# videosegmentation/video_segment

Hardware: AMD Instinct MI355X
Metric: over-segmented frames/sec at 1080p (higher is better)
Workload: dtype f32

## Files before the change

include/vsg.h:

```cpp
#ifndef VSG_H_
#define VSG_H_

#include <stddef.h>
#include <stdint.h>

#ifdef __cplusplus
extern "C" {
#endif

#define VSG_OK 0
#define VSG_ERR_INVALID -1
#define VSG_ERR_DEVICE -2
#define VSG_ERR_STATE -3
#define VSG_ERR_INTERNAL -4

#define VSG_MEM_HOST 0
#define VSG_MEM_DEVICE 1

typedef struct vsg_stream vsg_stream;
typedef struct vsg_graph vsg_graph;

typedef struct vsg_options {
  int presmoothing;
  float frac_min_region_size;
// ... 16 lines not shown
  float readout_ms;
  float host_post_ms;
  int64_t edges_total;
  int64_t edges_active;
  int64_t merges;
  int64_t preprocess_launches;
  int64_t edge_launches;
  float wave_kernel_ms;
  int64_t wave_kernel_launches;
  int64_t wave_kernel_edges;
  float filter_kernel_ms;
  int64_t filter_kernel_launches;
  float spine_kernel_ms;
  int64_t spine_kernel_launches;
  int64_t spine_kernel_edges;
} vsg_timings;

typedef struct vsg_diagnostics {
  double segment_wall_ms;
  double prepare_ms;
  double constrained_merge_ms;
  int64_t stages;
  int64_t optimistic_stages, rollbacks;
  int64_t slab_growths;
  double slab_growth_ms;
  int64_t spine_pool_growths;
  double spine_pool_growth_ms;
  int64_t runtime_mallocs;
  double runtime_malloc_ms;
  int64_t runtime_frees;
  double runtime_free_ms;
  int64_t cache_hits;
  int64_t device_syncs;
  double device_sync_ms;
  int64_t mail_waits;
  double mail_wait_ms;
  double mail_wait_longest_ms;
  int mail_mode;
} vsg_diagnostics;

typedef struct vsg_merge_paths {
  int64_t hub_stages;
  int64_t hub_absorbed;
  int64_t hub_cuts;
  int64_t hub_cuts_in_groups;
  int64_t hub_parts_in_later_bucket;
  int64_t spine_side_cuts;
  int64_t hub_retries;
  int64_t hub_reasons[6];
  int64_t hub_exclusion_reruns;
  int64_t hub_off_reruns;
  int64_t group_halvings;
  int64_t conservative_replays;
} vsg_merge_paths;

typedef struct vsg_memory_stats {
  int64_t bytes_in_use;
  int64_t bytes_in_use_peak;
  int64_t bytes_cached;
  int64_t limit_bytes;
  int64_t runtime_mallocs, runtime_frees, cache_hits, device_syncs;
  double runtime_malloc_ms, runtime_free_ms, device_sync_ms;
} vsg_memory_stats;
int vsg_device_memory_stats(int device, vsg_memory_stats* out);
int vsg_device_memory_trim(int device);
int vsg_device_memory_limit(int device, int64_t bytes);

const char* vsg_last_error(void);
int vsg_version(void);
void vsg_default_options(vsg_options* o);
int vsg_device_count(void);

int vsg_vectorize_id_image(const int32_t* ids, int width, int height, const uint8_t** data,
                           size_t* len);

int vsg_stream_create(const vsg_options* o, int width, int height, vsg_stream** out);
void vsg_stream_destroy(vsg_stream* s);
int vsg_stream_process_frame(vsg_stream* s, int flush, const uint8_t* bgr, size_t stride,
                             const float* flow, int has_flow_stream, int mem, int* num_results);
int vsg_stream_chunk_size(const vsg_stream* s);
int vsg_stream_result_bytes(vsg_stream* s, int i, const uint8_t** data, size_t* len);
int vsg_stream_result_id_image(vsg_stream* s, int i, int32_t* out);
int vsg_stream_last_merge_stats(const vsg_stream* s, int64_t* forced_regular_small);
int vsg_stream_last_timings(const vsg_stream* s, vsg_timings* t);
int vsg_stream_last_diagnostics(const vsg_stream* s, vsg_diagnostics* d);
int vsg_stream_last_merge_paths(const vsg_stream* s, vsg_merge_paths* out);
int vsg_stream_last_smoothed(vsg_stream* s, float* out);

int vsg_stream_export_halo(vsg_stream* s, const int32_t** dev_labels_virtual,
                           const int32_t** dev_labels_constrained, int64_t scalars[4]);
int vsg_stream_import_halo(vsg_stream* s, const int32_t* labels_virtual,
                           const int32_t* labels_constrained, int mem, const int64_t scalars[4]);

int vsg_stream_expect_halo(vsg_stream* s);
int vsg_stream_restart(vsg_stream* s);

typedef struct vsg_chain vsg_chain;
int vsg_chain_create(int rank, int world, const char* id_file, uint64_t nonce, int device,
                     vsg_chain** out);
void vsg_chain_destroy(vsg_chain* c);
int vsg_chain_info(const vsg_chain* c, int* rank, int* world);
int vsg_chain_send_halo(vsg_chain* c, vsg_stream* from, int dst);
int vsg_chain_recv_halo(vsg_chain* c, vsg_stream* into, int src);
int vsg_chain_exchange_halo(vsg_chain* c, vsg_stream* from, int dst, vsg_stream* into, int src);

typedef struct vsg_regionseg vsg_regionseg;
// ... 72 lines not shown
```

video_segment_amd/_lib.py:

```python
import ctypes as C
import os
import subprocess

_HERE = os.path.dirname(os.path.abspath(__file__))
CSRC_DIR = os.path.join(_HERE, "csrc")
LIB_PATH = os.path.join(_HERE, "lib", "libvsg_hip.so")

VSG_OK = 0
VSG_ERR_INVALID, VSG_ERR_DEVICE, VSG_ERR_STATE, VSG_ERR_INTERNAL = -1, -2, -3, -4
VSG_MEM_HOST = 0
VSG_MEM_DEVICE = 1


class VsgOptions(C.Structure):
    _fields_ = [
        ("presmoothing", C.c_int),
        ("frac_min_region_size", C.c_float),
        ("chunk_size", C.c_int),
        ("chunk_overlap_ratio", C.c_float),
        ("num_constraint_frames", C.c_int),
        ("enforce_n4_connectivity", C.c_int),
        ("enforce_spatial_connectedness", C.c_int),
        ("color_distance", C.c_int),
        ("device", C.c_int),
# ... 1 lines not shown
        ("compute_vectorization", C.c_int),
    ]


class VsgTimings(C.Structure):
    _fields_ = [
        ("preprocess_ms", C.c_float),
        ("edges_ms", C.c_float),
        ("sort_ms", C.c_float),
        ("merge_ms", C.c_float),
        ("readout_ms", C.c_float),
        ("host_post_ms", C.c_float),
        ("edges_total", C.c_int64),
        ("edges_active", C.c_int64),
        ("merges", C.c_int64),
        ("preprocess_launches", C.c_int64),
        ("edge_launches", C.c_int64),
        ("wave_kernel_ms", C.c_float),
        ("wave_kernel_launches", C.c_int64),
        ("wave_kernel_edges", C.c_int64),
        ("filter_kernel_ms", C.c_float),
        ("filter_kernel_launches", C.c_int64),
        ("spine_kernel_ms", C.c_float),
        ("spine_kernel_launches", C.c_int64),
        ("spine_kernel_edges", C.c_int64),
    ]


class VsgDiagnostics(C.Structure):
    _fields_ = [
        ("segment_wall_ms", C.c_double), ("prepare_ms", C.c_double), ("constrained_merge_ms", C.c_double),
        ("stages", C.c_int64), ("optimistic_stages", C.c_int64), ("rollbacks", C.c_int64),
        ("slab_growths", C.c_int64), ("slab_growth_ms", C.c_double),
        ("spine_pool_growths", C.c_int64), ("spine_pool_growth_ms", C.c_double),
        ("runtime_mallocs", C.c_int64), ("runtime_malloc_ms", C.c_double),
        ("runtime_frees", C.c_int64), ("runtime_free_ms", C.c_double),
        ("cache_hits", C.c_int64), ("device_syncs", C.c_int64), ("device_sync_ms", C.c_double),
        ("mail_waits", C.c_int64), ("mail_wait_ms", C.c_double), ("mail_wait_longest_ms", C.c_double),
        ("mail_mode", C.c_int),
    ]

    def as_dict(self):
        return {k: getattr(self, k) for k, _ in self._fields_}


class VsgMergePaths(C.Structure):
    _fields_ = [
        ("hub_stages", C.c_int64), ("hub_absorbed", C.c_int64),
        ("hub_cuts", C.c_int64), ("hub_cuts_in_groups", C.c_int64), ("hub_parts_in_later_bucket", C.c_int64),
        ("spine_side_cuts", C.c_int64),
        ("hub_retries", C.c_int64), ("hub_reasons", C.c_int64 * 6),
        ("hub_exclusion_reruns", C.c_int64), ("hub_off_reruns", C.c_int64),
        ("group_halvings", C.c_int64), ("conservative_replays", C.c_int64),
    ]

    def as_dict(self):
        return {k: (list(getattr(self, k)) if k == "hub_reasons" else getattr(self, k)) for k, _ in self._fields_}


class VsgMemoryStats(C.Structure):
    _fields_ = [
        ("bytes_in_use", C.c_int64), ("bytes_in_use_peak", C.c_int64), ("bytes_cached", C.c_int64),
        ("limit_bytes", C.c_int64),
        ("runtime_mallocs", C.c_int64), ("runtime_frees", C.c_int64), ("cache_hits", C.c_int64),
        ("device_syncs", C.c_int64),
        ("runtime_malloc_ms", C.c_double), ("runtime_free_ms", C.c_double), ("device_sync_ms", C.c_double),
    ]

    def as_dict(self):
        return {k: getattr(self, k) for k, _ in self._fields_}


class VsgRegionOptions(C.Structure):
    _fields_ = [
        ("min_region_num", C.c_int), ("max_region_num", C.c_int),
        ("level_cutoff_fraction", C.c_float), ("small_region_penalizer", C.c_float),
        ("luminance_bins", C.c_int), ("color_bins", C.c_int), ("flow_bins", C.c_int),
        ("chunk_set_size", C.c_int), ("chunk_set_overlap", C.c_int), ("constraint_chunks", C.c_int),
        ("use_appearance", C.c_int), ("use_flow", C.c_int), ("use_size_penalizer", C.c_int),
        ("compute_vectorization", C.c_int), ("save_descriptors", C.c_int),
    ]


EXPORTED_SYMBOLS = [
    "vsg_last_error", "vsg_version", "vsg_default_options", "vsg_device_count",
    "vsg_device_memory_stats", "vsg_device_memory_trim", "vsg_device_memory_limit",
    "vsg_vectorize_id_image",
    "vsg_stream_create", "vsg_stream_destroy", "vsg_stream_process_frame", "vsg_stream_chunk_size",
    "vsg_stream_result_bytes", "vsg_stream_result_id_image", "vsg_stream_last_merge_stats",
    "vsg_stream_last_timings", "vsg_stream_last_diagnostics", "vsg_stream_last_merge_paths", "vsg_stream_last_smoothed", "vsg_stream_export_halo",
    "vsg_stream_import_halo", "vsg_stream_expect_halo", "vsg_stream_restart",
    "vsg_chain_create", "vsg_chain_destroy", "vsg_chain_info", "vsg_chain_send_halo",
    "vsg_chain_recv_halo", "vsg_chain_exchange_halo",
    "vsg_regionseg_default_options", "vsg_regionseg_create", "vsg_regionseg_destroy", "vsg_regionseg_process_frame",
    "vsg_regionseg_result_bytes", "vsg_bgr_to_lab",
    "vsg_graph_create", "vsg_graph_destroy", "vsg_graph_add_frame_bgr",
    "vsg_graph_add_frame_features", "vsg_graph_add_virtual_frame", "vsg_graph_add_temporal",
    "vsg_graph_finish_building", "vsg_graph_segment_spatially", "vsg_graph_segment", "vsg_graph_obtain_results",
    "vsg_graph_num_frames", "vsg_graph_num_regions", "vsg_graph_num_neighbor_links",
    "vsg_graph_region_sizes", "vsg_graph_index_image", "vsg_graph_get_regions",
    "vsg_graph_get_intervals", "vsg_graph_smoothed",
    "vsg_graph_spatial_buckets", "vsg_graph_temporal_buckets", "vsg_graph_node_roots",
    "vsg_graph_merge_stats", "vsg_graph_timings", "vsg_graph_diagnostics", "vsg_graph_merge_paths",
    "vsg_debug_sort_pairs", "vsg_debug_sort_pairs_timed",
]

# ... 118 lines not shown
```

video_segment_amd/csrc/capi.cpp:

```cpp
#include <algorithm>
#include <cstring>
#include <memory>
#include <string>
#include <vector>

#include <rccl/rccl.h>

#include <chrono>
#include <cstdio>
#include <fstream>
#include <thread>

#include "../../include/vsg.h"
#include "region_segmentation.h"
#include "stream.h"

namespace {

thread_local std::string g_last_error;

template <class F>
int Guard(F&& f) {
  try {
    f();
// ... 47 lines not shown
}

}

struct vsg_stream {
  int device = 0;
  std::unique_ptr<vsg::DenseSegmentationHip> impl;
  std::vector<int32_t> id_image;
};

struct vsg_regionseg {
  std::unique_ptr<vsg::RegionSegmentationHost> impl;
  int W = 0, H = 0;
};

struct vsg_graph {
  int device = 0;
  int W = 0, H = 0;
  size_t wh = 0;
  hipStream_t stream = nullptr;
  std::unique_ptr<vsg::DenseGraphHip> g;
  std::unique_ptr<vsg::Preprocessor> pre;
  std::vector<std::shared_ptr<vsg::DevBuf<float>>> feats;
  std::vector<std::shared_ptr<vsg::DevBuf<float>>> flows_dev;
  vsg::DevBuf<uint8_t> staging_bgr;
  vsg::DevBuf<float> staging_f32;
  vsg::DevBuf<int32_t> staging_ids;
  vsg_timings timings;
  std::vector<vsg_region> out_regions;
  std::vector<int32_t> out_nbr_ptr, out_nbr_idx;
  std::vector<vsg_interval> out_intervals;
  ~vsg_graph() {
    if (stream) (void)hipStreamSynchronize(stream);
    g.reset();
    pre.reset();
    if (stream) (void)hipStreamDestroy(stream);
  }
};

static void FillMergePaths(const vsg::MergePaths& mp, vsg_merge_paths* o) {
  std::memset(o, 0, sizeof(*o));
  o->hub_stages = mp.hub_stages;
  o->hub_absorbed = mp.hub_absorbed;
  o->hub_cuts = mp.hub_cuts;
  o->hub_cuts_in_groups = mp.hub_cuts_in_groups;
  o->hub_parts_in_later_bucket = mp.hub_parts_in_later_bucket;
  o->spine_side_cuts = mp.spine_side_cuts;
  o->hub_retries = mp.hub_retries;
  for (int q = 0; q < 6; ++q) o->hub_reasons[q] = mp.hub_reasons[q];
  o->hub_exclusion_reruns = mp.hub_exclusion_reruns;
  o->hub_off_reruns = mp.hub_off_reruns;
  o->group_halvings = mp.group_halvings;
  o->conservative_replays = mp.conservative_replays;
}

static void FillDiagnostics(const vsg::GraphTimings& gt, vsg_diagnostics* d) {
  std::memset(d, 0, sizeof(*d));
  d->segment_wall_ms = gt.segment_wall_ms;
  d->prepare_ms = gt.prepare_ms;
  d->constrained_merge_ms = gt.constrained_merge_ms;
  d->stages = gt.stages;
  d->optimistic_stages = gt.optimistic_stages;
  d->rollbacks = gt.rollbacks;
  d->slab_growths = gt.slab_growths;
  d->slab_growth_ms = gt.slab_growth_ms;
  d->spine_pool_growths = gt.spine_growths;
  d->spine_pool_growth_ms = gt.spine_growth_ms;
  d->runtime_mallocs = gt.runtime_mallocs;
  d->runtime_malloc_ms = gt.runtime_malloc_ms;
  d->runtime_frees = gt.runtime_frees;
  d->runtime_free_ms = gt.runtime_free_ms;
  d->cache_hits = gt.cache_hits;
  d->device_syncs = gt.device_syncs;
  d->device_sync_ms = gt.device_sync_ms;
  d->mail_waits = gt.mail_waits;
  d->mail_wait_ms = gt.mail_wait_ms;
  d->mail_wait_longest_ms = gt.mail_wait_longest_ms;
  d->mail_mode = gt.mail_mode;
}

extern "C" {

const char* vsg_last_error(void) { return g_last_error.c_str(); }

int vsg_device_memory_stats(int device, vsg_memory_stats* out) {
  return Guard([&] {
    VSG_REQUIRE(out, VSG_ERR_INVALID, "null argument");
    const int dev = ResolveDevice(device);
    const vsg::CacheStats s = vsg::CacheGetStats(dev);
    out->bytes_in_use = s.bytes_in_use;
    out->bytes_in_use_peak = s.bytes_in_use_peak;
    out->bytes_cached = s.bytes_cached;
    out->limit_bytes = s.limit_bytes;
    out->runtime_mallocs = s.runtime_mallocs;
    out->runtime_frees = s.runtime_frees;
    out->cache_hits = s.cache_hits;
    out->device_syncs = s.device_syncs;
    out->runtime_malloc_ms = s.runtime_malloc_ms;
    out->runtime_free_ms = s.runtime_free_ms;
    out->device_sync_ms = s.device_sync_ms;
  });
}

int vsg_device_memory_trim(int device) {
  return Guard([&] {
    const int dev = ResolveDevice(device);
// ... 858 lines not shown
```

video_segment_amd/csrc/dense_graph.cpp:

```cpp
#include "dense_graph.h"
#include "scan_device.h"

#include <algorithm>
#include <chrono>
#include <cmath>
#include <cstring>
#include <atomic>
#include <functional>
#include <thread>
#include <unordered_set>

namespace vsg {

namespace {
template <class T>
DevBuf<T>& Grow(DevBuf<T>& b, size_t n) {
  if (b.size() < n) b.alloc(n + n / 2 + 1024);
  return b;
}
double NowMs() {
  using clk = std::chrono::steady_clock;
  return std::chrono::duration<double, std::milli>(clk::now().time_since_epoch()).count();
}
template <class T>
// ... 425 lines not shown
    if (getenv("VSG_DEBUG_STATS")) {
      std::fprintf(stderr, "[vsg] stage scratch: %zu -> %zu active edges (needed %lld), %.2f ms\n", before,
                   scratch_active_, need, NowMs() - tg0);
    }
    return true;
  };
  S.num_active = scalars_.get();
  S.num_segs = scalars_.get() + 1;
  S.node_key_bits = 1;
  while (S.node_key_bits < 32 && ((size_t)1 << S.node_key_bits) < N) ++S.node_key_bits;
  {
    const size_t words = 4 * ((scratch_edges_ + 255) / 256) + 4;
    S.masks.active = filter_masks_.get();
    S.masks.settled = filter_masks_.get() + words;
    S.masks.tentative = filter_masks_.get() + 2 * words;
    S.masks.block_cnt = block_cnt_.get();
    S.block_off = block_off_.get();
  }
  S.force_rollback = getenv("VSG_FORCE_ROLLBACK") ? 1 : 0;
  S.small_seg = getenv("VSG_SMALL_SEG") ? std::max(1, atoi(getenv("VSG_SMALL_SEG"))) : 24;
  S.wide_min = getenv("VSG_WIDE_MIN") ? atoi(getenv("VSG_WIDE_MIN")) : 0;
  S.wide_waves = getenv("VSG_WIDE_WAVES") ? atoi(getenv("VSG_WIDE_WAVES")) : 4;
  S.chain_relax = getenv("VSG_CHAIN_RELAX") ? atoi(getenv("VSG_CHAIN_RELAX")) : 1;
  const int hubs_default = getenv("VSG_HUBS") ? atoi(getenv("VSG_HUBS")) : 1;
  S.hubs = hubs_default;
  S.hub_excl = hub_excl_.get();
  S.hub_max_splits = getenv("VSG_HUB_SPLITS") ? std::max(0, atoi(getenv("VSG_HUB_SPLITS"))) : kHubMaxSplits;
  S.hub_cut_min_work = getenv("VSG_CUT_MIN_WORK") ? atoi(getenv("VSG_CUT_MIN_WORK")) : 0;
  S.hub_cut_ratio = getenv("VSG_CUT_RATIO") ? std::max(0, atoi(getenv("VSG_CUT_RATIO"))) : 1500;
  S.hub_check = (getenv("VSG_HUB_CHECK") && atoi(getenv("VSG_HUB_CHECK")) != 0) ? 1 : 0;
  VSG_HIP(hipMemsetAsync(hub8_.get(), 0, N, stream_));
  S.spine_min = getenv("VSG_SPINE_MIN") ? atoi(getenv("VSG_SPINE_MIN")) : 2048;
  {
    const double want = 1.15 * (double)wh_ * (double)capacity_frames_;
    const int by_graph = (int)std::min<double>(std::max<double>(want, 1 << 20), 120 << 20);
    S.spine_max_edges = getenv("VSG_SPINE_MAX_EDGES") ? atoi(getenv("VSG_SPINE_MAX_EDGES"))
                                                      : std::max(by_graph, spine_max_edges_grown_);
  }
  S.spine_off = 0;
  if (spine_limit_bucket_ != 0x7fffffff && ++spine_limit_age_ > 8) {
    spine_limit_bucket_ = 0x7fffffff;
    spine_limit_age_ = 0;
  }
  S.spine_limit_bucket = &spine_limit_bucket_;
  int spine_low_failed[2] = {0, 0}, spine_low_skip[2] = {0, 0};
  for (int b = 0; b < 2; ++b) {
    if (spine_low_cooldown_[b] > 0) {
      --spine_low_cooldown_[b];
      spine_low_skip[b] = 1;
    }
  }
  S.spine_low_failed = spine_low_failed;
  S.spine_low_skip = spine_low_skip;
  S.spine_nested_factor = getenv("VSG_SPINE_NESTED") ? std::max(1, atoi(getenv("VSG_SPINE_NESTED"))) : 1;
  S.spine_debug = getenv("VSG_SPINE_DEBUG") ? 1 : 0;
  S.spine_check = getenv("VSG_SPINE_CHECK") ? 1 : 0;
  S.rank_split_min = getenv("VSG_RANK_SPLIT_MIN") ? atoi(getenv("VSG_RANK_SPLIT_MIN")) : (1 << 20);
  S.spine_fast = getenv("VSG_SPINE_FAST") ? atoi(getenv("VSG_SPINE_FAST")) : 2;
  S.spine_fast_min = getenv("VSG_SPINE_FAST_MIN") ? atoi(getenv("VSG_SPINE_FAST_MIN")) : 32768;
  if (S.spine_min > 0) {
    const size_t ints = SpinePoolInts((size_t)S.spine_max_edges);
    if (spine_pool_.size() < ints) spine_pool_.alloc(ints);
  }
  S.spine_pool = spine_pool_.get();
  S.spine_pool_ints = spine_pool_.size();
  S.grow_spine_pool = [this, &S, &diag_spine_growths, &diag_spine_ms](long long edges) {
    if (getenv("VSG_SPINE_MAX_EDGES") || edges >= (120ll << 20)) return false;
    const long long want = std::min<long long>(edges + edges / 8, 120ll << 20);
    const long long nodes = (long long)wh_ * (long long)std::max(capacity_frames_, 1);
    const size_t ints = SpinePoolInts((size_t)want) + (size_t)(29 * std::min(want, nodes));
    if (ints <= spine_pool_.size()) return false;
    const double tg0 = NowMs();
    size_t free_b = 0, total_b = 0;
    VSG_HIP(hipMemGetInfo(&free_b, &total_b));
    if (free_b + spine_pool_.size() * sizeof(int32_t) < 2 * ints * sizeof(int32_t)) {
      int dev = 0;
      VSG_HIP(hipGetDevice(&dev));
      CacheTrim(dev);
      VSG_HIP(hipMemGetInfo(&free_b, &total_b));
      if (free_b + spine_pool_.size() * sizeof(int32_t) < 2 * ints * sizeof(int32_t)) return false;
    }
    VSG_HIP(hipStreamSynchronize(stream_));
    VSG_HIP(hipStreamSynchronize(aux_stream_));
    VSG_HIP(hipStreamSynchronize(aux2_stream_));
    spine_pool_.alloc(ints);
    ++diag_spine_growths;
    diag_spine_ms += NowMs() - tg0;
    S.spine_pool = spine_pool_.get();
    S.spine_pool_ints = spine_pool_.size();
    S.spine_max_edges = (int)want;
    spine_max_edges_grown_ = S.spine_max_edges;
    return true;
  };
  S.nmap[0] = label_uf_.get();
  S.nmap[1] = label_img_.get();
  S.nmap[2] = adjust_.get();
  S.aux_stream = aux_stream_;
  S.aux2_stream = aux2_stream_;
  S.aux_fork = aux_fork_;
  S.aux_join = aux_join_;
  S.use_rle = getenv("VSG_RLE") ? atoi(getenv("VSG_RLE")) : 1;
  S.wave_dbg = getenv("VSG_WAVE_DBG") ? atoi(getenv("VSG_WAVE_DBG")) : 0;
  S.wave_debug = (S.wave_dbg != 0 || getenv("VSG_DEBUG_STAGES") || getenv("VSG_DEBUG_STATS")) ? 1 : 0;
  optimistic_stages_ = 0;
  rollbacks_ = 0;
  S.optimistic_stages = &optimistic_stages_;
  S.rollbacks = &rollbacks_;
// ... 272 lines not shown
                 (long long)diag_hub_stages, (long long)diag_hub_absorbed, S.hub_splits, S.hub_retries, S.hub_reasons[0],
                 S.hub_reasons[1], S.hub_reasons[2], S.hub_reasons[3], S.hub_reasons[4], S.hub_reasons[5]);
    std::fprintf(stderr, "[vsg] wide: edges %llu batches %llu (%.1f lanes each) rounds %llu (%.1f per batch), chain lanes %llu, "
                 "kept-lane iterations %llu; kcyc per batch: staging %.1f rounds %.1f (%.2f per round)\n",
                 st[31], st[45], (double)st[72] / std::max(1.0, (double)st[45]), st[44],
                 (double)st[44] / std::max(1.0, (double)st[45]), st[73], st[74],
                 st[46] / 1e3 / std::max(1.0, (double)st[45]), st[47] / 1e3 / std::max(1.0, (double)st[45]),
                 st[47] / 1e3 / std::max(1.0, (double)st[44]));
  }
  timings_.merge_ms = (float)(NowMs() - t0);
  for (auto& pr : ev_wave_) {
    float ms = 0;
    VSG_HIP(hipEventElapsedTime(&ms, ev_pool_[pr.first], ev_pool_[pr.second]));
    timings_.wave_ms += ms;
  }
  for (auto& pr : ev_filter_) {
    float ms = 0;
    VSG_HIP(hipEventElapsedTime(&ms, ev_pool_[pr.first], ev_pool_[pr.second]));
    timings_.filter_ms += ms;
  }
  for (auto& pr : ev_spine_) {
    float ms = 0;
    VSG_HIP(hipEventElapsedTime(&ms, ev_pool_[pr.first], ev_pool_[pr.second]));
    timings_.spine_ms += ms;
  }
  timings_.spine_launches += (int64_t)ev_spine_.size();
  timings_.spine_edges += (int64_t)st[24];
  timings_.wave_launches += (int64_t)ev_wave_.size();
  timings_.filter_launches += (int64_t)ev_filter_.size();
  timings_.wave_edges += (int64_t)st[3];
  timings_.edges_active += (int64_t)st[3];
  timings_.edges_total = edges_total;
  timings_.merges[0] += (int64_t)st[0];
  timings_.merges[1] += (int64_t)st[1];
  timings_.merges[2] += (int64_t)st[2];
  {
    const ThreadAllocCounters a1 = ThreadAllocSnapshot();
    const MailWaitCounters m1 = MailWaitSnapshot();
    timings_.stages = diag_stages;
    MergePaths& mp = timings_.paths;
    mp = MergePaths();
    mp.hub_stages = diag_hub_stages;
    mp.hub_absorbed = diag_hub_absorbed;
    mp.hub_cuts = S.hub_splits;
    mp.hub_cuts_in_groups = S.hub_cuts_in_groups;
    mp.hub_parts_in_later_bucket = S.hub_parts_in_later_bucket;
    mp.spine_side_cuts = S.spine_side_cuts;
    mp.hub_retries = S.hub_retries;
    for (int q = 0; q < 6; ++q) mp.hub_reasons[q] = S.hub_reasons[q];
    mp.hub_exclusion_reruns = S.hub_exclusion_reruns;
    mp.hub_off_reruns = S.hub_off_reruns;
    mp.group_halvings = S.group_halvings;
    mp.conservative_replays = S.conservative_replays;
    timings_.slab_growths = diag_slab_growths;
    timings_.slab_growth_ms = diag_slab_ms;
    timings_.spine_growths = diag_spine_growths;
    timings_.spine_growth_ms = diag_spine_ms;
    timings_.runtime_mallocs = a1.runtime_mallocs - alloc0.runtime_mallocs;
    timings_.runtime_malloc_ms = a1.runtime_malloc_ms - alloc0.runtime_malloc_ms;
    timings_.runtime_frees = a1.runtime_frees - alloc0.runtime_frees;
    timings_.runtime_free_ms = a1.runtime_free_ms - alloc0.runtime_free_ms;
    timings_.cache_hits = a1.cache_hits - alloc0.cache_hits;
    timings_.device_syncs = a1.device_syncs - alloc0.device_syncs;
    timings_.device_sync_ms = a1.device_sync_ms - alloc0.device_sync_ms;
    timings_.mail_waits = m1.waits - mail0.waits;
    timings_.mail_wait_ms = m1.wait_ms - mail0.wait_ms;
    timings_.mail_wait_longest_ms = m1.longest_ms;
    timings_.mail_mode = MailYieldMode();
    timings_.prepare_ms = t0 - t_enter;
    timings_.constrained_merge_ms = t_mc - t_buckets;
    timings_.segment_wall_ms = NowMs() - t_enter;
  }
}

namespace {
struct SimRegion {
  int parent;
  float d[3];
  int sz, cons, flags;
  bool dirty;
};
}

void DenseGraphHip::DebugHash(const char* where) {
  const size_t N = wh_ * (size_t)num_frames_;
  std::vector<int32_t> parent(N), cons(N);
  std::vector<float4> ds(N);
  std::vector<uint8_t> flags(N);
  D2H(parent.data(), parent_.get(), N, stream_);
  D2H(cons.data(), cons_.get(), N, stream_);
  D2H(ds.data(), desc_sz_.get(), N, stream_);
  D2H(flags.data(), flags_.get(), N, stream_);
  VSG_HIP(hipStreamSynchronize(stream_));
  auto fnv = [](uint64_t h, const void* p, size_t n) {
    const uint8_t* b = static_cast<const uint8_t*>(p);
    for (size_t i = 0; i < n; ++i) { h ^= b[i]; h *= 1099511628211ull; }
    return h;
  };
  std::vector<int32_t> root(N), canon(N, -1);
  uint64_t h_part = 1469598103934665603ull, h_root = h_part, h_state = h_part, h_cons = h_part;
  int next = 0, nroots = 0;
  for (size_t i = 0; i < N; ++i) {
    int r = (int)i;
    while (parent[(size_t)r] != r) r = parent[(size_t)r];
    root[i] = r;
    if (canon[(size_t)r] < 0) canon[(size_t)r] = next++;
// ... 837 lines not shown
```

video_segment_amd/csrc/dense_graph.h:

```cpp
#ifndef VSG_DENSE_GRAPH_H_
#define VSG_DENSE_GRAPH_H_

#include <memory>
#include <unordered_map>
#include <vector>

#include "device_graph.h"
#include "host_model.h"

namespace vsg {

struct MergePaths {
  int64_t hub_stages = 0, hub_absorbed = 0;
  int64_t hub_cuts = 0, hub_cuts_in_groups = 0, hub_parts_in_later_bucket = 0, spine_side_cuts = 0;
  int64_t hub_retries = 0, hub_reasons[6] = {0, 0, 0, 0, 0, 0};
  int64_t hub_exclusion_reruns = 0, hub_off_reruns = 0, group_halvings = 0, conservative_replays = 0;
};

struct GraphTimings {
  float edges_ms = 0, sort_ms = 0, merge_ms = 0, readout_ms = 0, host_post_ms = 0;
  int64_t edges_total = 0, edges_active = 0;
  int64_t merges[3] = {0, 0, 0};
  float wave_ms = 0, filter_ms = 0, spine_ms = 0;
  int64_t wave_launches = 0, filter_launches = 0, wave_edges = 0, spine_launches = 0, spine_edges = 0;
  int64_t optimistic_stages = 0, rollbacks = 0;
  int64_t stages = 0;
  int64_t slab_growths = 0, spine_growths = 0;
  double slab_growth_ms = 0, spine_growth_ms = 0;
  int64_t runtime_mallocs = 0, runtime_frees = 0, cache_hits = 0, device_syncs = 0;
  double runtime_malloc_ms = 0, runtime_free_ms = 0, device_sync_ms = 0;
  int64_t mail_waits = 0;
  double mail_wait_ms = 0, mail_wait_longest_ms = 0;
  int mail_mode = 0;
  double segment_wall_ms = 0, prepare_ms = 0, constrained_merge_ms = 0;
  MergePaths paths;
};

class DenseGraphHip {
 public:
  DenseGraphHip(int W, int H, int max_frames, bool l1, hipStream_t stream);
  ~DenseGraphHip();

  int W() const { return W_; }
  int H() const { return H_; }
  int max_frames() const { return max_frames_; }
  int num_frames() const { return num_frames_; }
  hipStream_t stream() const { return stream_; }

  void Reset(int max_frames);
  void ForgetLearned();

  void AddFrame(const float* feat_planar_dev, const int32_t* cons_dev);
  void AddVirtualFrame(const int32_t* ids_dev, int max_label);
  void AddVirtualFrameDeferred();
  void SetHaloLabels(const int32_t* virtual_ids_dev, const int32_t* constrained_ids_dev,
                     int max_label);
  bool halo_pending() const { return halo_pending_; }
  void AddTemporal(const float* cur_dev, const float* prev_dev, const float* flow_dev,
                   bool is_virtual);
  void FinishBuilding();
  void Segment(int min_region_size, bool force_constraints) {
    SegmentLists(min_region_size, force_constraints, spatial_pass_done_ ? 2 : 0);
  }
  void SegmentSpatially() {
    SegmentLists(0, false, 1);
    spatial_pass_done_ = true;
  }
  void ObtainResults(const std::vector<const float*>* dev_flows, bool enforce_n4,
                     bool enforce_spatial_connectedness);
// ... 144 lines not shown
```

video_segment_amd/csrc/device_graph.h:

```cpp
#ifndef VSG_DEVICE_GRAPH_H_
#define VSG_DEVICE_GRAPH_H_

#include <functional>

#include "common.h"

namespace vsg {

constexpr uint8_t kFlagFinalized = 1;
constexpr uint8_t kFlagNoDesc = 2;
constexpr uint8_t kFlagTentative = 4;
constexpr uint8_t kFlagHub = 8;
constexpr uint8_t kFlagHubBroken = 16;
constexpr uint8_t kFlagHubExcluded = 32;
constexpr int kHubExclCap = 16384;
constexpr int kHubMaxAttempts = 4;
constexpr int kHubMaxSplits = 64;
constexpr int kHubCutCap = 64;
constexpr int kHubListInts = 4 + kHubExclCap + 3 * kHubCutCap;

struct NodeArrays {
  int32_t* parent;
  float4* desc_sz;
  int32_t* cons;
// ... 117 lines not shown
  unsigned long long* tentative;
  int32_t* block_cnt;
};
struct FilterSegs {
  const int32_t* start;
  const int32_t* list;
  const int32_t* pos0;
  int n;
};
struct MergeScratch {
  int active_cap;
  std::function<bool(long long need)> grow_active;
  int32_t* e_ra;
  int32_t* e_rb;
  uint32_t* e_gpos;
  int32_t* e_active;
  int32_t* e_apos;
  FilterMasks masks;
  int32_t* block_off;
  int32_t* a_ra;
  int32_t* a_rb;
  uint32_t* a_gpos;
  uint32_t* a_comp;
  uint32_t* a_idx;
  uint32_t* s_comp;
  uint32_t* s_idx;
  uint32_t* seg_key;
  int32_t* seg_cnt;
  int32_t* seg_off;
  int32_t* num_active;
  int32_t* num_segs;
  float4* bk_ds;
  int32_t* bk_cons;
  uint8_t* bk_flags;
  int force_rollback;
  int32_t* lead_pos;
  int32_t* l_ra;
  int32_t* l_rb;
  uint32_t* l_gpos;
  int use_rle;
  int group_hi;
  const int32_t* bucket_prefix;
  const int32_t* bucket_prefix_host;
  const int32_t* bucket_base_host;
  const int32_t* list_off_host;
  int32_t* seg_dev;
  size_t seg_cap;
  std::vector<int32_t>* seg_host;
  int spine_min;
  int spine_off;
  int* spine_low_failed;
  const int* spine_low_skip;
  int* spine_limit_bucket;
  int spine_nested_factor;
  int spine_max_edges;
  int spine_debug, spine_check;
  int rank_split_min;
  int spine_fast;
  int spine_fast_min;
  int32_t* spine_pool;
  size_t spine_pool_ints;
  std::function<bool(long long edges)> grow_spine_pool;
  int32_t* nmap[3];
  hipStream_t aux_stream;
  hipStream_t aux2_stream;
  hipEvent_t aux_fork, aux_join;
  int small_seg;
  int wide_min;
  int wide_waves;
  int chain_relax;
  int hubs;
  int hubs_off;
  int hub_attempt;
  int hub_splits_left;
  int hub_split_depth;
  int hub_list_dirty;
  int hub_max_splits;
  int hub_cut_min_work;
  long long hub_splits;
  const uint32_t* list_slot_base_host;
  int32_t* hub_excl;
  long long hub_retries;
  long long hub_reasons[6];
  long long hub_cuts_in_groups;
  long long hub_parts_in_later_bucket;
  long long spine_side_cuts;
  long long hub_exclusion_reruns;
  long long hub_off_reruns;
  long long group_halvings;
  long long conservative_replays;
  long long hub_cut_ratio;
  int hub_check;
  int wave_debug;
  int wave_dbg;
  int64_t* optimistic_stages;
  int64_t* rollbacks;
  int32_t* cc;
  unsigned long long* stats;
  void* cub_temp;
  size_t cub_temp_bytes;
  ScanScratch scan;
  int node_key_bits;
  std::vector<hipEvent_t>* ev_pool;
  std::vector<std::pair<int, int>>* ev_wave;
  std::vector<std::pair<int, int>>* ev_filter;
  std::vector<std::pair<int, int>>* ev_spine;
  int* ev_used;
  Mailbox* mail;
  ZeroPool* zeros;
  hipStream_t main_stream;
};
int32_t* TakeZeroed(MergeScratch& S, size_t n);

int32_t* TakeStageScalars(MergeScratch& S, size_t n);

void LaunchBuildBucketTable(const ListDesc* lists, int num_lists, int32_t* bucket_base,
                            hipStream_t s);
void LaunchInitIdentity(int32_t* a, size_t n, hipStream_t s);
struct StageInfo {
  int want_components = 0;
  int replayed = 0;
  int components = 0;
  int max_wave_segment = 0;
  int hub_stages = 0;
  long long hub_absorbed = 0;
  int hub_retries = 0;
};
void ResetHubExclusions(MergeScratch& S, NodeArrays nodes, hipStream_t s);
void RunBucketStage(int bucket, int j0, int n_b, const ListDesc* lists, const int32_t* bucket_base,
                    const uint32_t* list_slot_base, uint8_t* kept_all, NodeArrays nodes,
                    const MergeParams& P, int inert_mode, MergeScratch& S, hipStream_t s,
                    StageInfo* info = nullptr);
size_t SpinePoolInts(size_t max_edges);
void LaunchKeepVirtualBucket(const ListDesc* lists, int num_lists, hipStream_t s);

void LaunchFlatten(NodeArrays nodes, size_t n, int32_t* label_uf, hipStream_t s);
void LaunchEnforceN4(int32_t* label_img, int W, int H, const int32_t* frames_dev, int num_frames,
                     int32_t* row_flags , int32_t* adjust ,
                     hipStream_t s);
void LaunchRowRunCounts(const int32_t* label_img, int W, int H, int frame, int32_t* row_counts,
                        hipStream_t s);
struct IntervalArrays {
  int32_t* label;
// ... 48 lines not shown
```

video_segment_amd/csrc/merge_common.h:

```cpp
#ifndef VSG_MERGE_COMMON_H_
#define VSG_MERGE_COMMON_H_

#include <functional>
#include <vector>

#include "device_graph.h"

namespace vsg {

constexpr int kSmallSegment = 24;
constexpr int kTabDirty = 0x100;

__device__ __forceinline__ int FindCompress(int32_t* __restrict__ parent, int x) {
  int root = x;
  int p = parent[root];
  while (p != root) {
    root = p;
    p = parent[root];
  }
  int cur = x;
  while (cur != root) {
    const int next = parent[cur];
    if (next != root) parent[cur] = root;
    cur = next;
// ... 293 lines not shown
  o = max(o, Dpp0<0x118, 0xf, 0xc>(o));
  o = max(o, Dpp0<0x142, 0xa, 0xf>(o));
  o = max(o, Dpp0<0x143, 0xc, 0xf>(o));
  return __builtin_amdgcn_readlane(o, 63);
}

struct WorkerArgs {
  const int32_t* num_segs;
  const int32_t* seg_off;
  const int32_t* seg_cnt;
  const int32_t* s_ra;
  const int32_t* s_rb;
  const uint32_t* s_gpos;
  NodeArrays nodes;
  uint8_t* kept_all;
  StageThr T;
  int optimistic;
  int32_t* violation;
  unsigned long long* stats;
  int small_seg;
  int wave_min;
  int wave_max;
  uint32_t* work_list;
  int work_cap;
  int32_t* work_ctl;
  int wide_min = 0;
  int wide_waves = 4;
  int32_t* hub_mark = nullptr;
  const uint32_t* s_seq = nullptr;
  int32_t* hub_excl = nullptr;
};
constexpr int kWaveClasses = 3;
constexpr int kWaveClassMin1 = 192;
constexpr int kWaveClassMin0 = 1536;
void LaunchMergeWave(int grid, const WorkerArgs& a, bool instrumented, int dbg_flags, hipStream_t s);
void LaunchMergeWide(int grid, const WorkerArgs& a, int waves, hipStream_t s);

inline int NextEvent(MergeScratch& S) {
  if (!S.ev_pool) return -1;
  if (*S.ev_used >= (int)S.ev_pool->size()) {
    hipEvent_t e;
    VSG_HIP(hipEventCreate(&e));
    S.ev_pool->push_back(e);
  }
  return (*S.ev_used)++;
}

struct SpineSeg {
  int off;
  int cnt;
};
struct SpineInput {
  std::vector<SpineSeg> segs;
};
using SpineWorkers = std::function<void(const WorkerArgs&, int n_edges, hipStream_t)>;
constexpr int kSpineListCap = 4095;
int SelectLargeSegments(int max_segs, const int32_t* num_segs, const int32_t* seg_off, const int32_t* seg_cnt,
                        int min_cnt, long long max_edges, MergeScratch& S, hipStream_t s, SpineInput* out,
                        long long* wanted_edges);
bool RunSpineComponents(const SpineInput& in, const WorkerArgs& wa, MergeScratch& S, hipStream_t s,
                        const SpineWorkers& run_workers, size_t pool_used, int depth);

}

#endif
```

video_segment_amd/csrc/merge_spine.hip:

```cpp
#include <algorithm>
#include <chrono>
#include <cstdlib>
#include <cstdio>
#include <unordered_map>
#include <vector>

#include "merge_common.h"
#include "scan_device.h"

namespace vsg {

namespace {

constexpr int kNone = -1;

static inline unsigned Blocks(size_t n) { return (unsigned)((n + 255) / 256); }

__device__ __forceinline__ int CompOf(const int32_t* __restrict__ comp_base, int K, int e) {
  int lo = 0, hi = K;
  while (hi - lo > 1) {
    const int mid = (lo + hi) >> 1;
    if (comp_base[mid] <= e) lo = mid; else hi = mid;
  }
  return lo;
}

__global__ __launch_bounds__(256) void k_spine_gather(int mE, int K, const int32_t* __restrict__ comp_base,
                                                       const int32_t* __restrict__ comp_off,
                                                       const int32_t* __restrict__ s_ra,
                                                       const int32_t* __restrict__ s_rb,
                                                       int32_t* __restrict__ eu, int32_t* __restrict__ ev,
                                                       int32_t* __restrict__ estate, int32_t* __restrict__ cc,
                                                       uint32_t* __restrict__ best) {
  const int e = blockIdx.x * 256 + threadIdx.x;
  const bool valid = e < mE;
  int u = -1, v = -1;
  if (valid) {
    const int lo = CompOf(comp_base, K, e);
    const int pos = comp_off[lo] + (e - comp_base[lo]);
    u = s_ra[pos];
    v = s_rb[pos];
    eu[e] = u;
    ev[e] = v;
    estate[e] = 0;
  }
  const int pu = __shfl_up(u, 1), pv = __shfl_up(v, 1);
  const bool first = (threadIdx.x & 63) == 0;
  if (valid && (first || (u != pu && u != pv))) {
    cc[u] = u;
    best[u] = 0xffffffffu;
  }
  if (valid && v != u && (first || (v != pu && v != pv))) {
    cc[v] = v;
    best[v] = 0xffffffffu;
  }
}

constexpr int kAliveSlots = 32;
__device__ __forceinline__ uint32_t BorKey(int round, int e) { return ((uint32_t)(31 - round) << 27) | (uint32_t)e; }

__global__ __launch_bounds__(256) void k_bor_min(int n, const int32_t* __restrict__ list,
                                                  const int32_t* __restrict__ list_len, int round,
                                                  const int32_t* __restrict__ eu,
                                                  const int32_t* __restrict__ ev, int32_t* __restrict__ estate,
                                                  int32_t* __restrict__ cc, uint32_t* __restrict__ best,
                                                  int32_t* __restrict__ ecu, int32_t* __restrict__ ecv,
                                                  int32_t* __restrict__ alive, const int32_t* __restrict__ gate,
                                                  int32_t* __restrict__ next_len) {
  if (blockIdx.x == 0 && threadIdx.x == 0) *next_len = 0;
  if (gate && *gate == 0) return;
  const int i = blockIdx.x * 256 + threadIdx.x;
  if (list_len) n = min(n, *list_len);
  const int e = i < n ? (list ? list[i] : i) : -1;
  bool live = false;
  int cu = -1, cv = -1;
  if (e >= 0 && round == 0) {
    cu = eu[e];
    cv = ev[e];
    live = true;
  } else if (e >= 0 && estate[e] == 0) {
    cu = CcFind(cc, eu[e]);
    cv = CcFind(cc, ev[e]);
    if (cu == cv) {
      estate[e] = 2;
      cu = cv = -1;
    } else {
      live = true;
      ecu[e] = cu;
      ecv[e] = cv;
    }
  }
  const int pu = __shfl_up(cu, 1), pv = __shfl_up(cv, 1), pe = __shfl_up(e, 1);
  if (live) {
    const uint32_t key = BorKey(round, e);
    const bool has_prev = (threadIdx.x & 63) != 0 && pe < e;
    if (!(has_prev && (cu == pu || cu == pv)) && key < best[cu]) atomicMin(&best[cu], key);
    if (!(has_prev && (cv == pu || cv == pv)) && key < best[cv]) atomicMin(&best[cv], key);
  }
// ... 1116 lines not shown
    sum += group;
    taken = j;
    thr = sizes[(size_t)i];
    i = j;
  }
  if (taken == 0) return 0x7fffffff;
  for (int i = 0; i < found; ++i) {
    if (large[2 + 2 * i] >= thr) out->segs.push_back(SpineSeg{large[1 + 2 * i], large[2 + 2 * i]});
  }
  return thr;
}

bool RunSpineComponents(const SpineInput& in, const WorkerArgs& wa, MergeScratch& S, hipStream_t s,
                        const SpineWorkers& run_workers, size_t pool_used, int depth) {
  const int K = (int)in.segs.size();
  if (K == 0) return false;
  std::vector<int32_t> base(K + 1, 0), off(K);
  for (int k = 0; k < K; ++k) {
    base[k + 1] = base[k] + in.segs[k].cnt;
    off[k] = in.segs[k].off;
  }
  const int mE = base[K];
  VSG_REQUIRE(mE < (1 << 27), -4, "spine: too many edges for the stamped ranks");
  double tph[8] = {0};
  auto Mark = [&](int i) {
    if (!S.spine_debug) return;
    VSG_HIP(hipStreamSynchronize(s));
    tph[i] = std::chrono::duration<double, std::milli>(std::chrono::steady_clock::now().time_since_epoch()).count();
  };
  Mark(0);
  if (pool_used >= S.spine_pool_ints) return false;
  Pool pool{S.spine_pool + pool_used, S.spine_pool_ints - pool_used};
  int32_t* d_base = pool.take(K + 1);
  int32_t* d_off = pool.take(K);
  int32_t* root_vertex = pool.take(K);
  int32_t* comp_spine = pool.take(K + 1);
  unsigned long long* root_key = reinterpret_cast<unsigned long long*>(TakeZeroed(S, 2 * (size_t)K));
  int32_t* scalars = pool.take(64);
  int32_t* eu = pool.take(mE);
  int32_t* ev = pool.take(mE);
  int32_t* estate = pool.take(mE);
  int32_t* flag = pool.take(mE);
  int32_t* scan = pool.take(mE);
  int32_t* side_key = pool.take(mE);
  int32_t* spine_flag = pool.take(mE);
  if (!pool.ok) return false;
  int32_t* cc = S.cc;
  uint32_t* best = reinterpret_cast<uint32_t*>(S.nmap[0]);
  int32_t* firstq = S.nmap[1];
  int32_t* childidx = S.nmap[2];

  VSG_HIP(hipMemcpyAsync(d_base, base.data(), (K + 1) * sizeof(int32_t), hipMemcpyHostToDevice, s));
  VSG_HIP(hipMemcpyAsync(d_off, off.data(), K * sizeof(int32_t), hipMemcpyHostToDevice, s));
  hipLaunchKernelGGL(k_spine_gather, dim3(Blocks(mE)), dim3(256), 0, s, mE, K, d_base, d_off, wa.s_ra,
                     wa.s_rb, eu, ev, estate, cc, best);
  hipLaunchKernelGGL(k_spine_pick_root, dim3(Blocks((size_t)K + (mE + kRootStride - 1) / kRootStride)), dim3(256), 0,
                     s, mE, K, eu, ev, d_base, wa.nodes, root_key);
  hipLaunchKernelGGL(k_spine_roots, dim3((K + 63) / 64), dim3(64), 0, s, K, root_key, root_vertex, childidx);

  int dbg_rounds = 0;
  auto NowMs = [] {
    return std::chrono::duration<double, std::milli>(std::chrono::steady_clock::now().time_since_epoch()).count();
  };
  const bool dbg_big = S.spine_debug && mE > (8 << 20);
  if (dbg_big) {
    VSG_HIP(hipStreamSynchronize(s));
    std::fprintf(stderr, "[vsg]   forest: gather+root %.2f ms\n", NowMs() - tph[0]);
  }
  {
    const size_t forest_mark = pool.mark();
    const int32_t* list = nullptr;
    const int32_t* list_len = nullptr;
    int n_list = mE;
    int32_t* lists[2] = {nullptr, nullptr};
    int which = 0;
    const int ahead_max = getenv("VSG_BOR_AHEAD") ? atoi(getenv("VSG_BOR_AHEAD")) : (4 << 20);
    const int compact_min = getenv("VSG_BOR_COMPACT_MIN") ? atoi(getenv("VSG_BOR_COMPACT_MIN")) : (1 << 16);
    MailSlot waiting[2];
    int n_waiting = 0;
    const int32_t* gate = nullptr;
    int32_t* len_words = scalars + 8;
    int32_t* gate_words = scalars + 12;
    int len_cur = 0;
    for (int round = 0;; ++round) {
      dbg_rounds = round;
      VSG_REQUIRE(round < 32, -4, "spine: the spanning forest did not converge");
      int32_t* d_ctr = TakeZeroed(S, 16 * kAliveSlots + 4);
      int32_t* d_next_len = len_words + (len_cur ^ 1);
      hipLaunchKernelGGL(k_bor_min, dim3(Blocks(n_list)), dim3(256), 0, s, n_list, list, list_len, round, eu, ev,
                         estate, cc, best, side_key, spine_flag, d_ctr, gate, d_next_len);
      const MailSlot m_alive = NextMail(*S.mail);
      hipLaunchKernelGGL(k_bor_hook, dim3(Blocks(n_list)), dim3(256), 0, s, n_list, list, list_len, round, eu, ev,
                         estate, cc, best, side_key, spine_flag, d_ctr, m_alive.dev, m_alive.seq, gate,
                         gate_words + (round & 1));
      gate = gate_words + (round & 1);
      waiting[n_waiting++] = m_alive;
      const int depth = n_list <= ahead_max ? 1 : 0;
      const double tr0 = dbg_big ? NowMs() : 0;
      int alive = -1;
      bool complete = false;
      while (n_waiting > depth) {
        MailWait(waiting[0], 1, &alive, s);
        waiting[0] = waiting[1];
        --n_waiting;
        if (alive == 0) {
          complete = true;
          break;
        }
      }
      if (dbg_big) std::fprintf(stderr, "[vsg]   forest round %d: %d in list, %d alive, %.2f ms\n", round, n_list, alive, NowMs() - tr0);
      if (complete) break;
      const bool compact = depth == 1 ? (round >= 1 && n_list > compact_min)
                                      : (alive < n_list / 2 && n_list > compact_min);
      if (!compact) continue;
      if (!lists[0]) {
        const size_t m = pool.mark();
        const size_t cap = depth == 1 ? (size_t)n_list : (size_t)alive;
        lists[0] = pool.take(cap);
        lists[1] = pool.take(cap);
        if (!pool.ok) {
          pool.ok = true;
          pool.release(m);
// ... 112 lines not shown
  pool.release(arcs_mark);
  const MailSlot m_side = NextMail(*S.mail);
  FusedScan(S.scan, ScanLoadI32{flag}, FlagScanEmit{nullptr, scan}, TotalPostFinish{scalars + 2, m_side.dev, m_side.seq},
            mE, s);
  int n_side = 0;
  MailWait(m_side, 1, &n_side, s);
  const size_t ns = (size_t)(n_side > 0 ? n_side : 1);
  uint32_t* sk_in = reinterpret_cast<uint32_t*>(pool.take(ns));
  uint32_t* si_in = reinterpret_cast<uint32_t*>(pool.take(ns));
  uint32_t* sk = reinterpret_cast<uint32_t*>(pool.take(ns));
  uint32_t* si = reinterpret_cast<uint32_t*>(pool.take(ns));
  uint32_t* seg_key = reinterpret_cast<uint32_t*>(pool.take(ns));
  int32_t* seg_cnt = pool.take(ns);
  int32_t* seg_off = pool.take(ns);
  int32_t* o_ra = pool.take(ns);
  int32_t* o_rb = pool.take(ns);
  uint32_t* o_gpos = reinterpret_cast<uint32_t*>(pool.take(ns));
  if (!pool.ok) return false;
  hipLaunchKernelGGL(k_compact_side, dim3(Blocks(mE)), dim3(256), 0, s, mE, flag, scan, side_key, sk_in, si_in);
  FusedScan(S.scan, StateFlagValue{spine_flag, 1}, SpineEmit{eu, ev, childidx, te_e, scan, sp_child, sp_is_a, d_base, d_off, K},
            SpineFinish{comp_spine, K}, mE, s);
  hipLaunchKernelGGL(k_comp_spine, dim3(Blocks(K)), dim3(256), 0, s, K, d_base, scan, comp_spine);
  int dbg_spine_edges = 0;
  if (S.spine_debug) {
    std::vector<int32_t> cs(K + 1);
    VSG_HIP(hipMemcpy(cs.data(), comp_spine, (K + 1) * sizeof(int32_t), hipMemcpyDeviceToHost));
    dbg_spine_edges = cs[K];
  }
  Mark(4);
  if (S.spine_check) SpineSelfCheck(base, mE, eu, ev, root_vertex, side_key, spine_flag, te_e, mt);
  if (n_side > 0) {
    int side_bits = 1;
    while (side_bits < 32 && (1ll << side_bits) < (long long)mt) ++side_bits;
    SortPairsU32(S.cub_temp, S.cub_temp_bytes, sk_in, sk, si_in, si, n_side, side_bits, s);
    int32_t* d_nseg = scalars + 3;
    RunsOfSortedKeys(S.scan, sk, n_side, seg_off, seg_cnt, d_nseg, s);
    hipLaunchKernelGGL(k_gather_side, dim3(Blocks(n_side)), dim3(256), 0, s, n_side, si, d_base, d_off, K, wa.s_ra,
                       wa.s_rb, wa.s_gpos, o_ra, o_rb, o_gpos);
    WorkerArgs w2 = wa;
    w2.num_segs = d_nseg;
    w2.seg_off = seg_off;
    w2.seg_cnt = seg_cnt;
    w2.s_ra = o_ra;
    w2.s_rb = o_rb;
    w2.s_gpos = o_gpos;
    w2.T.side = 1;
    w2.s_seq = nullptr;
    VSG_REQUIRE(w2.T.hubs == 0, -4, "tree replay: a side cluster in a stage with hub regions");
    w2.work_cap = n_side / (w2.small_seg + 1) + 1;
    w2.work_list = (size_t)kWaveClasses * w2.work_cap <= ns ? seg_key : nullptr;
    w2.work_ctl = w2.work_list ? TakeZeroed(S, 2 * kWaveClasses) : nullptr;
    SpineInput nested;
    w2.wave_max = 0x7fffffff;
    if (pool.ok && depth < 8 && n_side >= S.spine_min * S.spine_nested_factor) {
      const long long room = (long long)((S.spine_pool_ints - pool_used - pool.used) / 16);
      w2.wave_max = SelectLargeSegments(n_side, d_nseg, seg_off, seg_cnt, S.spine_min * S.spine_nested_factor,
                                        room < S.spine_max_edges ? room : S.spine_max_edges, S, s, &nested,
                                        nullptr);
    }
    if (nested.segs.empty()) {
      run_workers(w2, n_side, s);
    } else {
      const int ef = NextEvent(S), ej = NextEvent(S);
      const bool fork = S.aux2_stream && ef >= 0 && ej >= 0;
      if (fork) {
        VSG_HIP(hipEventRecord((*S.ev_pool)[ef], s));
        VSG_HIP(hipStreamWaitEvent(S.aux2_stream, (*S.ev_pool)[ef], 0));
        run_workers(w2, n_side, S.aux2_stream);
        VSG_HIP(hipEventRecord((*S.ev_pool)[ej], S.aux2_stream));
      } else {
        run_workers(w2, n_side, s);
      }
      if (!RunSpineComponents(nested, w2, S, s, run_workers, pool_used + pool.used, depth + 1)) {
        WorkerArgs w3 = w2;
        w3.wave_min = w2.wave_max - 1;
        w3.wave_max = 0x7fffffff;
        w3.work_list = nullptr;
        run_workers(w3, n_side, s);
      }
      if (fork) VSG_HIP(hipStreamWaitEvent(s, (*S.ev_pool)[ej], 0));
    }
  }
  Mark(5);
  const int es0 = NextEvent(S);
  if (es0 >= 0) VSG_HIP(hipEventRecord((*S.ev_pool)[es0], s));
  int32_t* start_pos = nullptr;
  const auto LaunchSpine = [&](int max_steps) {
    hipLaunchKernelGGL(k_spine, dim3(K), dim3(64 * (1 + kSpineReaders)), 0, s, K, comp_spine, root_vertex, sp_child,
                       sp_is_a, wa.nodes, wa.T, wa.optimistic, wa.violation, wa.stats, start_pos, max_steps,
                       wa.s_gpos, wa.hub_excl);
  };
  if (S.spine_fast > 0 && mt >= S.spine_fast_min) {
    SpineFastArrays F;
    F.ck_stride = (mt >> 4) + 2 * K + 4;
    F.p = pool.take(mt);
    F.ds = reinterpret_cast<float4*>(pool.take(4 * (size_t)mt));
    F.meta = pool.take(mt);
    F.sizes = pool.take((size_t)mt + 1);
    F.pre = pool.take((size_t)mt + 1);
    F.ck = reinterpret_cast<float*>(pool.take(3 * (size_t)F.ck_stride));
    F.stop = pool.take(K);
    F.fail = pool.take(K);
    F.start_pos = pool.take(K);
    if (pool.ok) {
      start_pos = F.start_pos;
      for (int pass = 0; pass < S.spine_fast; ++pass) {
        if (pass > 0) LaunchSpine(64);
        hipLaunchKernelGGL(k_spine_fast_init, dim3((K + 63) / 64), dim3(64), 0, s, K, comp_spine, F, pass == 0 ? 1 : 0);
        hipLaunchKernelGGL(k_spine_prep, dim3(Blocks((size_t)mt + 1)), dim3(256), 0, s, mt, K, comp_spine,
                           root_vertex, sp_child, wa.nodes, wa.T, F);
        ExclusiveSum(S.scan, F.sizes, F.pre, mt + 1, s);
        hipLaunchKernelGGL(k_spine_chain, dim3(K), dim3(64 * (1 + kChProducers)), 0, s, K, comp_spine, root_vertex,
                           wa.nodes, F);
        hipLaunchKernelGGL(k_spine_verify, dim3(Blocks((size_t)F.ck_stride)), dim3(256), 0, s, K, comp_spine,
                           root_vertex, wa.nodes, wa.T, F);
        hipLaunchKernelGGL(k_spine_commit, dim3(Blocks(((size_t)mt + kCommitPer - 1) / kCommitPer)), dim3(256), 0, s, mt, K, comp_spine, root_vertex,
                           wa.nodes, F, wa.stats);
        hipLaunchKernelGGL(k_spine_finish, dim3((K + 63) / 64), dim3(64), 0, s, K, comp_spine, root_vertex,
                           wa.nodes, wa.T, F, wa.stats);
        if (S.spine_debug) {
          VSG_HIP(hipStreamSynchronize(s));
          std::vector<int32_t> cs(K + 1), sp(K), st(K), fl(K);
          VSG_HIP(hipMemcpy(cs.data(), comp_spine, (K + 1) * sizeof(int32_t), hipMemcpyDeviceToHost));
          VSG_HIP(hipMemcpy(sp.data(), F.start_pos, K * sizeof(int32_t), hipMemcpyDeviceToHost));
          VSG_HIP(hipMemcpy(st.data(), F.stop, K * sizeof(int32_t), hipMemcpyDeviceToHost));
          VSG_HIP(hipMemcpy(fl.data(), F.fail, K * sizeof(int32_t), hipMemcpyDeviceToHost));
          long long total = 0, fast = 0;
          int longest = 0, stopped = 0, failed = 0;
          for (int k = 0; k < K; ++k) {
            const int n = cs[k + 1] - cs[k];
            total += n;
            fast += sp[k];
            longest = std::max(longest, n);
            stopped += st[k] < n;
            failed += fl[k] < n;
          }
          std::fprintf(stderr, "[vsg]   streamed chain, pass %d: %lld of %lld spine steps done (longest spine %d; %d of %d "
                       "components stopped at a step that is not plain, %d at a failed test or a larger side "
                       "cluster)\n", pass, fast, total, longest, stopped, K, failed);
        }
      }
    }
  }
  LaunchSpine(0x7fffffff);
  const int es1 = NextEvent(S);
  if (es1 >= 0) {
    VSG_HIP(hipEventRecord((*S.ev_pool)[es1], s));
    if (S.ev_spine) S.ev_spine->emplace_back(es0, es1);
  }
  VSG_HIP(hipGetLastError());
  Mark(6);
  if (S.spine_debug) {
    std::fprintf(stderr, "[vsg] spine[%d]: %d components, %d edges (largest %d), %d tree edges, %d side edges, %d spine edges, "
                 "%d boruvka rounds | ms: forest %.2f rooting %.2f paths %.2f classify %.2f side %.2f spine %.2f\n",
                 depth, K, mE, in.segs[0].cnt, mt, n_side, dbg_spine_edges, dbg_rounds, tph[1] - tph[0], tph[2] - tph[1],
                 tph[3] - tph[2], tph[4] - tph[3], tph[5] - tph[4], tph[6] - tph[5]);
  }
  return true;
}

}
```

Measured before the change: 202.3.

## Inherit spanning forest state in nested spine levels instead of recomputing Boruvka

Nested spine components now receive the parent level's edge state and side-index map. The gather kernel then marks each edge as tree or non-tree from the parent forest, and the Boruvka spanning-forest rounds are skipped for that level. This removes repeated forest construction (many rounds and launches) on nested side clusters. It depends on the parent forest restricted to the nested segment still being a valid spanning forest. A new nested-minimum knob and inheritance counters are also added.

After: 204.4, median of 3. About the same (+1.0%).

```diff
diff --git a/include/vsg.h b/include/vsg.h
--- a/include/vsg.h
+++ b/include/vsg.h
@@ -92,6 +92,8 @@
   int64_t hub_off_reruns;
   int64_t group_halvings;
   int64_t conservative_replays;
+  int64_t spine_levels;
+  int64_t spine_levels_inherited;
 } vsg_merge_paths;
 
 typedef struct vsg_memory_stats {
diff --git a/video_segment_amd/_lib.py b/video_segment_amd/_lib.py
--- a/video_segment_amd/_lib.py
+++ b/video_segment_amd/_lib.py
@@ -77,6 +77,7 @@
         ("hub_retries", C.c_int64), ("hub_reasons", C.c_int64 * 6),
         ("hub_exclusion_reruns", C.c_int64), ("hub_off_reruns", C.c_int64),
         ("group_halvings", C.c_int64), ("conservative_replays", C.c_int64),
+        ("spine_levels", C.c_int64), ("spine_levels_inherited", C.c_int64),
     ]
 
     def as_dict(self):
diff --git a/video_segment_amd/csrc/capi.cpp b/video_segment_amd/csrc/capi.cpp
--- a/video_segment_amd/csrc/capi.cpp
+++ b/video_segment_amd/csrc/capi.cpp
@@ -123,6 +123,8 @@
   o->hub_off_reruns = mp.hub_off_reruns;
   o->group_halvings = mp.group_halvings;
   o->conservative_replays = mp.conservative_replays;
+  o->spine_levels = mp.spine_levels;
+  o->spine_levels_inherited = mp.spine_levels_inherited;
 }
 
 static void FillDiagnostics(const vsg::GraphTimings& gt, vsg_diagnostics* d) {
diff --git a/video_segment_amd/csrc/dense_graph.cpp b/video_segment_amd/csrc/dense_graph.cpp
--- a/video_segment_amd/csrc/dense_graph.cpp
+++ b/video_segment_amd/csrc/dense_graph.cpp
@@ -501,7 +501,9 @@
   }
   S.spine_low_failed = spine_low_failed;
   S.spine_low_skip = spine_low_skip;
-  S.spine_nested_factor = getenv("VSG_SPINE_NESTED") ? std::max(1, atoi(getenv("VSG_SPINE_NESTED"))) : 1;
+  S.spine_nested_min = S.spine_min * (getenv("VSG_SPINE_NESTED") ? std::max(1, atoi(getenv("VSG_SPINE_NESTED"))) : 1);
+  if (getenv("VSG_SPINE_NESTED_MIN")) S.spine_nested_min = std::max(2, atoi(getenv("VSG_SPINE_NESTED_MIN")));
+  S.spine_inherit = getenv("VSG_SPINE_INHERIT") ? (atoi(getenv("VSG_SPINE_INHERIT")) != 0 ? 1 : 0) : 1;
   S.spine_debug = getenv("VSG_SPINE_DEBUG") ? 1 : 0;
   S.spine_check = getenv("VSG_SPINE_CHECK") ? 1 : 0;
   S.rank_split_min = getenv("VSG_RANK_SPLIT_MIN") ? atoi(getenv("VSG_RANK_SPLIT_MIN")) : (1 << 20);
@@ -880,6 +882,8 @@
     mp.hub_off_reruns = S.hub_off_reruns;
     mp.group_halvings = S.group_halvings;
     mp.conservative_replays = S.conservative_replays;
+    mp.spine_levels = S.spine_levels;
+    mp.spine_levels_inherited = S.spine_levels_inherited;
     timings_.slab_growths = diag_slab_growths;
     timings_.slab_growth_ms = diag_slab_ms;
     timings_.spine_growths = diag_spine_growths;
diff --git a/video_segment_amd/csrc/dense_graph.h b/video_segment_amd/csrc/dense_graph.h
--- a/video_segment_amd/csrc/dense_graph.h
+++ b/video_segment_amd/csrc/dense_graph.h
@@ -15,6 +15,7 @@
   int64_t hub_cuts = 0, hub_cuts_in_groups = 0, hub_parts_in_later_bucket = 0, spine_side_cuts = 0;
   int64_t hub_retries = 0, hub_reasons[6] = {0, 0, 0, 0, 0, 0};
   int64_t hub_exclusion_reruns = 0, hub_off_reruns = 0, group_halvings = 0, conservative_replays = 0;
+  int64_t spine_levels = 0, spine_levels_inherited = 0;
 };
 
 struct GraphTimings {
diff --git a/video_segment_amd/csrc/device_graph.h b/video_segment_amd/csrc/device_graph.h
--- a/video_segment_amd/csrc/device_graph.h
+++ b/video_segment_amd/csrc/device_graph.h
@@ -193,7 +193,8 @@
   int* spine_low_failed;
   const int* spine_low_skip;
   int* spine_limit_bucket;
-  int spine_nested_factor;
+  int spine_nested_min;
+  int spine_inherit;
   int spine_max_edges;
   int spine_debug, spine_check;
   int rank_split_min;
@@ -230,6 +231,8 @@
   long long hub_off_reruns;
   long long group_halvings;
   long long conservative_replays;
+  long long spine_levels;
+  long long spine_levels_inherited;
   long long hub_cut_ratio;
   int hub_check;
   int wave_debug;
diff --git a/video_segment_amd/csrc/merge_common.h b/video_segment_amd/csrc/merge_common.h
--- a/video_segment_amd/csrc/merge_common.h
+++ b/video_segment_amd/csrc/merge_common.h
@@ -369,6 +369,8 @@
 };
 struct SpineInput {
   std::vector<SpineSeg> segs;
+  const int32_t* parent_estate = nullptr;
+  const uint32_t* parent_si = nullptr;
 };
 using SpineWorkers = std::function<void(const WorkerArgs&, int n_edges, hipStream_t)>;
 constexpr int kSpineListCap = 4095;
diff --git a/video_segment_amd/csrc/merge_spine.hip b/video_segment_amd/csrc/merge_spine.hip
--- a/video_segment_amd/csrc/merge_spine.hip
+++ b/video_segment_amd/csrc/merge_spine.hip
@@ -31,7 +31,9 @@
                                                        const int32_t* __restrict__ s_rb,
                                                        int32_t* __restrict__ eu, int32_t* __restrict__ ev,
                                                        int32_t* __restrict__ estate, int32_t* __restrict__ cc,
-                                                       uint32_t* __restrict__ best) {
+                                                       uint32_t* __restrict__ best,
+                                                       const int32_t* __restrict__ parent_estate,
+                                                       const uint32_t* __restrict__ parent_si) {
   const int e = blockIdx.x * 256 + threadIdx.x;
   const bool valid = e < mE;
   int u = -1, v = -1;
@@ -42,8 +44,9 @@
     v = s_rb[pos];
     eu[e] = u;
     ev[e] = v;
-    estate[e] = 0;
-  }
+    estate[e] = parent_estate ? (parent_estate[parent_si[pos]] == 1 ? 1 : 2) : 0;
+  }
+  if (parent_estate) return;
   const int pu = __shfl_up(u, 1), pv = __shfl_up(v, 1);
   const bool first = (threadIdx.x & 63) == 0;
   if (valid && (first || (u != pu && u != pv))) {
@@ -1266,8 +1269,10 @@
 
   VSG_HIP(hipMemcpyAsync(d_base, base.data(), (K + 1) * sizeof(int32_t), hipMemcpyHostToDevice, s));
   VSG_HIP(hipMemcpyAsync(d_off, off.data(), K * sizeof(int32_t), hipMemcpyHostToDevice, s));
+  const bool inherit = S.spine_inherit && in.parent_estate && in.parent_si;
   hipLaunchKernelGGL(k_spine_gather, dim3(Blocks(mE)), dim3(256), 0, s, mE, K, d_base, d_off, wa.s_ra,
-                     wa.s_rb, eu, ev, estate, cc, best);
+                     wa.s_rb, eu, ev, estate, cc, best, inherit ? in.parent_estate : nullptr,
+                     inherit ? in.parent_si : nullptr);
   hipLaunchKernelGGL(k_spine_pick_root, dim3(Blocks((size_t)K + (mE + kRootStride - 1) / kRootStride)), dim3(256), 0,
                      s, mE, K, eu, ev, d_base, wa.nodes, root_key);
   hipLaunchKernelGGL(k_spine_roots, dim3((K + 63) / 64), dim3(64), 0, s, K, root_key, root_vertex, childidx);
@@ -1281,7 +1286,7 @@
     VSG_HIP(hipStreamSynchronize(s));
     std::fprintf(stderr, "[vsg]   forest: gather+root %.2f ms\n", NowMs() - tph[0]);
   }
-  {
+  if (!inherit) {
     const size_t forest_mark = pool.mark();
     const int32_t* list = nullptr;
     const int32_t* list_len = nullptr;
@@ -1500,11 +1505,13 @@
     w2.work_ctl = w2.work_list ? TakeZeroed(S, 2 * kWaveClasses) : nullptr;
     SpineInput nested;
     w2.wave_max = 0x7fffffff;
-    if (pool.ok && depth < 8 && n_side >= S.spine_min * S.spine_nested_factor) {
+    if (pool.ok && depth < 8 && n_side >= S.spine_nested_min) {
       const long long room = (long long)((S.spine_pool_ints - pool_used - pool.used) / 16);
-      w2.wave_max = SelectLargeSegments(n_side, d_nseg, seg_off, seg_cnt, S.spine_min * S.spine_nested_factor,
+      w2.wave_max = SelectLargeSegments(n_side, d_nseg, seg_off, seg_cnt, S.spine_nested_min,
                                         room < S.spine_max_edges ? room : S.spine_max_edges, S, s, &nested,
                                         nullptr);
+      nested.parent_estate = estate;
+      nested.parent_si = si;
     }
     if (nested.segs.empty()) {
       run_workers(w2, n_side, s);
@@ -1604,6 +1611,8 @@
                  depth, K, mE, in.segs[0].cnt, mt, n_side, dbg_spine_edges, dbg_rounds, tph[1] - tph[0], tph[2] - tph[1],
                  tph[3] - tph[2], tph[4] - tph[3], tph[5] - tph[4], tph[6] - tph[5]);
   }
+  ++S.spine_levels;
+  if (inherit) ++S.spine_levels_inherited;
   return true;
 }
 
```
